# frgfm/Holocron

Hardware: NVIDIA H100
Metric: images/sec RepVGG-A0 224^2 bf16 train (higher is better)
Workload: dtype bf16

## Files before the change

### holocron_b200/_lib.py

```python
import ctypes
import os
from pathlib import Path
from typing import Optional

import torch

_LIB_PATH = Path(__file__).resolve().parent / "csrc" / "libholocron_b200.so"
_lib: Optional[ctypes.CDLL] = None

DTYPE_CODE = {torch.float32: 0, torch.bfloat16: 1, torch.float16: 2}


class HolocronB200Error(RuntimeError):
    pass


def lib_path() -> Path:
    return _LIB_PATH


SIGNATURES = {
    "hb_hard_mish_fwd": "ppzip",
    "hb_hard_mish_bwd": "pppzip",
    "hb_nl_relu_fwd": "ppzfip",
# ... 8 lines not shown
    "hb_conv2d_wgrad_acc_bf16": "ppppz" + "i" * 11 + "p",
    "hb_repvgg_wgrad_acc_bf16": "ppppppz" + "i" * 6 + "p",
    "hb_pack_conv_weights": "ppp" + "i" * 8 + "p",
    "hb_zero_insert_bf16": "pp" + "i" * 7 + "p",
    "hb_pack_conv_weights_multi": "ppip",
    "hb_pack_chunk_elems": "",
    "hb_pack_meta_bytes": "",
    "hb_conv2d_dgrad_s2_bf16": "ppppp" + "i" * 8 + "p",
    "hb_pack_dgrad_s2_weights": "pp" + "i" * 4 + "p",
    "hb_nchw_to_nhwc_pad_bf16": "pp" + "i" * 6 + "p",
    "hb_im2col_smallc_bf16": "pp" + "i" * 10 + "p",
    "hb_conv2d_fused_bf16": "ppp",
    "hb_conv_stat_slots_max": "",
    "hb_patch_stats_bf16": "pppp" + "i" * 10 + "fp",
    "hb_bn_stats_partials_bf16": "piippp",
    "hb_bn_stat_slots_max": "",
    "hb_bn_finalize": "ppppppp" + "pppp" + "iiiiffp",
    "hb_bn_partials_sums": "ppiiiipp",
    "hb_bn_finalize_sums": "p" * 10 + "iiiffp",
    "hb_bn_eval_affine": "ppppfiippppp",
    "hb_bn_act_fwd_bf16": "pppipppp" + "iiifi" + "ppp",
    "hb_bn_bwd_scratch_doubles": "iii",
    "hb_bn_act_bwd_bf16": "ppppi" + "pppppp" + "pppppp" + "pp" + "iiiifiip",
    "hb_bn_act_bwd_reduce_bf16": "ppppi" + "pppppp" + "pppp" + "iiiifip",
    "hb_bn_act_bwd_apply_bf16": "ppppi" + "pppppp" + "ppppp" + "iiifip",
    "hb_dwconv_fwd_bf16": "pppp" + "iiiiiiip",
    "hb_dwconv_bwd_data_bf16": "ppp" + "iiiiiiip",
    "hb_dwconv_wgrad_scratch_doubles": "ii",
    "hb_dwconv_bwd_weight_bf16": "ppppp" + "iiiiiiip",
    "hb_involution_fwd_bf16": "ppp" + "i" * 11 + "p",
# ... 138 lines not shown
```

### holocron_b200/csrc/bn_act.cu

```cuda
#include <cstdio>
#include <cstdlib>
#include <type_traits>
#include <utility>
#include "common.cuh"
#include "act.cuh"
#include "slab.cuh"

namespace {

using namespace hb;

constexpr int kThreads = kSlabThreads;
constexpr int kMaxBranches = 3;

struct Branches {
  const __nv_bfloat16* u[kMaxBranches];
  int n;
};

__device__ __forceinline__ void fold_stat_partials(const SlabGeo& g, const float* red, int C, float* parts) {
  fold_row_lanes<double, 2>(g, red, [&](int c, const double (&a)[2]) {
    *reinterpret_cast<float2*>(parts + ((size_t)blockIdx.x * C + c) * 2) = make_float2((float)a[0], (float)a[1]);
  });
}

__global__ void __launch_bounds__(kThreads) bn_stats_partials_kernel(const __nv_bfloat16* __restrict__ u, int M, int C,
                                                                     SlabGeo g, float* __restrict__ parts) {
  __shared__ float red[2][kThreads * 8];
  const auto [tx, ty, cg, active] = g.thread();
  float s[8], q[8];
#pragma unroll
  for (int j = 0; j < 8; ++j) { s[j] = 0.f; q[j] = 0.f; }
  if (active) {
    const size_t row_stride = (size_t)gridDim.x * g.rows_t;
    size_t m = (size_t)blockIdx.x * g.rows_t + ty;
    for (; m + row_stride < (size_t)M; m += 2 * row_stride) {
      float a[8], b[8];
      unpack8(ld16_stream(u + m * C + cg * 8), a);
      unpack8(ld16_stream(u + (m + row_stride) * C + cg * 8), b);
#pragma unroll
      for (int j = 0; j < 8; ++j) { s[j] += a[j] + b[j]; q[j] += a[j] * a[j] + b[j] * b[j]; }
    }
    if (m < (size_t)M) {
      float a[8];
      unpack8(ld16_stream(u + m * C + cg * 8), a);
#pragma unroll
      for (int j = 0; j < 8; ++j) { s[j] += a[j]; q[j] += a[j] * a[j]; }
    }
  }
#pragma unroll
  for (int j = 0; j < 8; ++j) { red[0][threadIdx.x * 8 + j] = s[j]; red[1][threadIdx.x * 8 + j] = q[j]; }
  __syncthreads();
  fold_stat_partials(g, &red[0][0], C, parts);
}

struct FinalizeParams {
  const float* parts[kMaxBranches];
  int slots[kMaxBranches];
  const float* gamma[kMaxBranches];
  const float* beta[kMaxBranches];
  float* running_mean[kMaxBranches];
  float* running_var[kMaxBranches];
  long long* num_batches_tracked[kMaxBranches];
  float* mean;
  float* rstd;
  float* scale;
  float* shift;
  int B, C, M;
// ... 137 lines not shown
  shift[c] = (beta ? beta[c] : 0.f) - rmean[c] * sc;
  if (mean) mean[c] = rmean[c];
  if (rstd) rstd[c] = r;
}

struct FwdParams {
  Branches br;
  const float* scale;
  const float* shift;
  const __nv_bfloat16* residual;
  __nv_bfloat16* out;
  int M, C, act;
  float slope;
  int res_after;
  float* out_stats;
};
using RawVec = Vec16<__nv_bfloat16>;

__device__ __forceinline__ void lds8(const float* p, float* f) {
  const float4 a = *reinterpret_cast<const float4*>(p);
  const float4 b = *reinterpret_cast<const float4*>(p + 4);
  f[0] = a.x; f[1] = a.y; f[2] = a.z; f[3] = a.w; f[4] = b.x; f[5] = b.y; f[6] = b.z; f[7] = b.w;
}

__host__ __device__ constexpr int ring_depth(int nt) { return nt <= 2 ? 7 : 3; }

__device__ __forceinline__ void cp_async16(uint32_t saddr, const void* g) {
  asm volatile("cp.async.cg.shared.global [%0], [%1], 16;" ::"r"(saddr), "l"(g) : "memory");
}
__device__ __forceinline__ void cp_async_commit() { asm volatile("cp.async.commit_group;" ::: "memory"); }
template <int N>
__device__ __forceinline__ void cp_async_wait() { asm volatile("cp.async.wait_group %0;" ::"n"(N) : "memory"); }
__device__ __forceinline__ RawVec lds16(uint32_t saddr) {
  RawVec r;
  asm volatile("ld.shared.v4.u32 {%0,%1,%2,%3}, [%4];" : "=r"(r.raw.x), "=r"(r.raw.y), "=r"(r.raw.z), "=r"(r.raw.w) : "r"(saddr));
  return r;
}
__device__ __forceinline__ uint32_t smem_addr(const void* p) { return (uint32_t)__cvta_generic_to_shared(p); }

template <int NT>
struct RowRing {
  static constexpr int kDepth = ring_depth(NT);
  static constexpr int kSlots = kDepth + 1;
  uint32_t base;
  size_t m0, stride, M;
  size_t col_off;
  int C;
  const __nv_bfloat16* src[NT > 0 ? NT : 1];
  __device__ __forceinline__ void init(uint8_t* smem, size_t m0_, size_t stride_, int M_, int C_, size_t col_off_) {
    base = smem_addr(smem) + threadIdx.x * 16;
    m0 = m0_; stride = stride_; M = (size_t)M_; col_off = col_off_; C = C_;
  }
  __device__ __forceinline__ uint32_t addr(int s, int t) const { return base + (uint32_t)((s * NT + t) * kThreads * 16); }
  __device__ __forceinline__ bool valid(size_t k) const { return m0 + k * stride < M; }
  __device__ __forceinline__ size_t off(size_t k) const { return (m0 + k * stride) * C + col_off; }
  __device__ __forceinline__ void issue(size_t k) const {
    if (valid(k)) {
      const int s = (int)(k % kSlots);
      const size_t o = off(k);
#pragma unroll
      for (int t = 0; t < NT; ++t)
        if (src[t]) cp_async16(addr(s, t), src[t] + o);
    }
    cp_async_commit();
  }
  __device__ __forceinline__ void prologue() const {
#pragma unroll
    for (int k = 0; k < kDepth; ++k) issue(k);
  }
  __device__ __forceinline__ void wait() const { cp_async_wait<kDepth - 1>(); }
};

template <int NB, bool kStats>
__global__ void __launch_bounds__(kThreads, 3) bn_act_fwd_kernel(FwdParams p, SlabGeo g) {
  extern __shared__ __align__(16) uint8_t ring_smem[];
  const auto [tx, ty, cg, active] = g.thread();
  float os[8], oq[8];
#pragma unroll
  for (int j = 0; j < 8; ++j) { os[j] = 0.f; oq[j] = 0.f; }
  __shared__ __align__(16) float k_sc[kMaxBranches][256];
  __shared__ __align__(16) float k_sh[256];
  {
    const int nch = g.cg_t * 8;
    for (int ch = threadIdx.x; ch < nch; ch += kThreads) {
      const int c = blockIdx.y * nch + ch;
      float shv = 0.f;
#pragma unroll
      for (int b = 0; b < NB; ++b) {
        k_sc[b][ch] = c < p.C ? p.scale[(size_t)b * p.C + c] : 0.f;
        shv += c < p.C ? p.shift[(size_t)b * p.C + c] : 0.f;
      }
      k_sh[ch] = shv;
    }
    __syncthreads();
  }
  if (!active && !kStats) return;
  if (active) {
    const bool has_res = p.residual != nullptr;
    RowRing<NB + 1> ring;
    ring.init(ring_smem, (size_t)blockIdx.x * g.rows_t + ty, (size_t)gridDim.x * g.rows_t, p.M, p.C, (size_t)cg * 8);
#pragma unroll
    for (int b = 0; b < NB; ++b) ring.src[b] = p.br.u[b];
    ring.src[NB] = p.residual;
    ring.prologue();
    for (size_t k = 0; ring.valid(k); ++k) {
      ring.wait();
      const int s = (int)(k % RowRing<NB + 1>::kSlots);
      RawVec u[NB > 0 ? NB : 1], r;
#pragma unroll
      for (int b = 0; b < NB; ++b) u[b] = lds16(ring.addr(s, b));
      if (has_res) r = lds16(ring.addr(s, NB));
      ring.issue(k + RowRing<NB + 1>::kDepth);
      float z[8];
      lds8(&k_sh[tx * 8], z);
#pragma unroll
      for (int b = 0; b < NB; ++b) {
        float f[8], sc[8];
        lds8(&k_sc[b][tx * 8], sc);
        unpack8(u[b], f);
#pragma unroll
        for (int j = 0; j < 8; ++j) z[j] = fmaf(sc[j], f[j], z[j]);
      }
      float rr[8];
      if (has_res) unpack8(r, rr);
      if (has_res && !p.res_after) {
        if (p.act == ACT_FRELU) {
#pragma unroll
          for (int j = 0; j < 8; ++j) z[j] = max_nan(z[j], rr[j]);
        } else {
#pragma unroll
          for (int j = 0; j < 8; ++j) z[j] += rr[j];
        }
      }
#pragma unroll
      for (int j = 0; j < 8; ++j) z[j] = act_fwd(p.act, z[j], p.slope);
      if (has_res && p.res_after) {
#pragma unroll
        for (int j = 0; j < 8; ++j) z[j] += rr[j];
      }
      Vec16<__nv_bfloat16> ov;
#pragma unroll
      for (int j = 0; j < 8; ++j) ov.v[j] = __float2bfloat16_rn(z[j]);
      st16(p.out + ring.off(k), ov);
      if (kStats) {
#pragma unroll
        for (int j = 0; j < 8; ++j) {
          const float f = __bfloat162float(ov.v[j]);
          os[j] += f; oq[j] = fmaf(f, f, oq[j]);
        }
      }
    }
  }
  if (!kStats) return;
  cp_async_wait<0>();
  __syncthreads();
  float* red = reinterpret_cast<float*>(ring_smem);
#pragma unroll
  for (int j = 0; j < 8; ++j) {
    red[threadIdx.x * 8 + j] = active ? os[j] : 0.f;
    red[kThreads * 8 + threadIdx.x * 8 + j] = active ? oq[j] : 0.f;
  }
  __syncthreads();
  fold_stat_partials(g, red, p.C, p.out_stats);
}

struct BwdParams {
  Branches br;
  const __nv_bfloat16* dout;
  const __nv_bfloat16* residual;
  const float* scale;
  const float* shift;
  const float* mean;
  const float* rstd;
  double* sums;
  double* part;
  const double* count;
  __nv_bfloat16* du[kMaxBranches];
  __nv_bfloat16* dres;
  int M, C, act;
  float slope;
  int train;
  int res_after;
};

struct SlabConsts {
  float scale[kMaxBranches][256];
  float cu[kMaxBranches][256];
  float c0[kMaxBranches][256];
  float shift[256];
};
// ... 56 lines not shown
#pragma unroll
      for (int j = 0; j < 8; ++j) {
        const float gate = z[j] > r[j] ? 1.f : (z[j] == r[j] ? 0.5f : 0.f);
        dz[j] = d[j] * gate;
        dr[j] = d[j] - dz[j];
      }
      return;
    }
#pragma unroll
    for (int j = 0; j < 8; ++j) z[j] += r[j];
  }
#pragma unroll
  for (int j = 0; j < 8; ++j) { dz[j] = d[j] * act_grad(p.act, z[j], p.slope); dr[j] = dz[j]; }
}

template <int NB>
__device__ __forceinline__ void init_bwd_ring(RowRing<NB + 2>& ring, const BwdParams& p, const SlabGeo& g, uint8_t* ring_smem,
                                              int ty, int cg) {
  ring.init(ring_smem, (size_t)blockIdx.x * g.rows_t + ty, (size_t)gridDim.x * g.rows_t, p.M, p.C, (size_t)cg * 8);
#pragma unroll
  for (int b = 0; b < NB; ++b) ring.src[b] = p.br.u[b];
  ring.src[NB] = (p.residual && !p.res_after) ? p.residual : nullptr;
  ring.src[NB + 1] = p.dout;
}

template <int NB>
__global__ void __launch_bounds__(kThreads, 2) bn_act_bwd_reduce_kernel(BwdParams p, SlabGeo g) {
  extern __shared__ __align__(16) uint8_t dyn_smem[];
  SlabConsts& k = *reinterpret_cast<SlabConsts*>(dyn_smem);
  float* red = reinterpret_cast<float*>(dyn_smem + sizeof(SlabConsts));
  uint8_t* ring_smem = dyn_smem + sizeof(SlabConsts) + kThreads * 8 * sizeof(float);
  load_slab_consts<NB>(k, p, g, false);
  const auto [tx, ty, cg, active] = g.thread();
  float acc[1 + NB][8];
#pragma unroll
  for (int i = 0; i < 1 + NB; ++i)
#pragma unroll
    for (int j = 0; j < 8; ++j) acc[i][j] = 0.f;
  if (active) {
    RowRing<NB + 2> ring;
    init_bwd_ring<NB>(ring, p, g, ring_smem, ty, cg);
    ring.prologue();
    for (size_t kk = 0; ring.valid(kk); ++kk) {
      ring.wait();
      const int s = (int)(kk % RowRing<NB + 2>::kSlots);
      RawVec uv[NB > 0 ? NB : 1], rv, dv;
#pragma unroll
      for (int b = 0; b < NB; ++b) uv[b] = lds16(ring.addr(s, b));
      if (ring.src[NB]) rv = lds16(ring.addr(s, NB));
      dv = lds16(ring.addr(s, NB + 1));
      ring.issue(kk + RowRing<NB + 2>::kDepth);
      float u[NB > 0 ? NB : 1][8], dz[8], dr[8];
      recompute_dz<NB>(p, k, tx * 8, uv, rv, dv, u, dz, dr);
#pragma unroll
      for (int j = 0; j < 8; ++j) acc[0][j] += dz[j];
#pragma unroll
      for (int b = 0; b < NB; ++b) {
#pragma unroll
        for (int j = 0; j < 8; ++j) acc[1 + b][j] = fmaf(dz[j], u[b][j], acc[1 + b][j]);
      }
    }
  }
#pragma unroll
  for (int i = 0; i < 1 + NB; ++i) {
    __syncthreads();
#pragma unroll
    for (int j = 0; j < 8; ++j) red[threadIdx.x * 8 + j] = acc[i][j];
    __syncthreads();
    fold_row_lanes<double, 1>(g, red, [&](int c, const double (&a)[1]) {
      p.part[((size_t)blockIdx.x * (1 + NB) + i) * p.C + c] = a[0];
    });
  }
}

template <int NB>
__global__ void __launch_bounds__(kThreads, 2) bn_act_bwd_apply_kernel(BwdParams p, SlabGeo g) {
  extern __shared__ __align__(16) uint8_t dyn_smem[];
  SlabConsts& k = *reinterpret_cast<SlabConsts*>(dyn_smem);
  uint8_t* ring_smem = dyn_smem + sizeof(SlabConsts);
  load_slab_consts<NB>(k, p, g, true);
  const auto [tx, ty, cg, active] = g.thread();
  if (!active) return;
  RowRing<NB + 2> ring;
  init_bwd_ring<NB>(ring, p, g, ring_smem, ty, cg);
  ring.prologue();
  for (size_t kk = 0; ring.valid(kk); ++kk) {
    ring.wait();
    const int s = (int)(kk % RowRing<NB + 2>::kSlots);
    RawVec uv[NB > 0 ? NB : 1], rv, dv;
#pragma unroll
    for (int b = 0; b < NB; ++b) uv[b] = lds16(ring.addr(s, b));
    if (ring.src[NB]) rv = lds16(ring.addr(s, NB));
    dv = lds16(ring.addr(s, NB + 1));
    ring.issue(kk + RowRing<NB + 2>::kDepth);
    const size_t off = ring.off(kk);
    float u[NB > 0 ? NB : 1][8], dz[8], dr[8];
    recompute_dz<NB>(p, k, tx * 8, uv, rv, dv, u, dz, dr);
    if (p.dres) store8(p.dres + off, dr);
#pragma unroll
    for (int b = 0; b < NB; ++b) {
      if (p.du[b]) {
        float sc[8], cu[8], c0[8], d[8];
        lds8(&k.scale[b][tx * 8], sc);
        lds8(&k.cu[b][tx * 8], cu);
        lds8(&k.c0[b][tx * 8], c0);
#pragma unroll
        for (int j = 0; j < 8; ++j) d[j] = fmaf(sc[j], dz[j], fmaf(cu[j], u[b][j], c0[j]));
        store8(p.du[b] + off, d);
      }
// ... 24 lines not shown
    const float db = (float)tot[0];
    if (p.dgamma) p.dgamma[o] = dg;
    if (p.dbeta) p.dbeta[o] = db;
    if (c < p.C_logical) {
      if (p.gacc[b]) p.gacc[b][c] += dg;
      if (p.bacc[b]) p.bacc[b][c] += db;
    }
  }
}

inline int env_int(const char* name, int dflt) {
  const char* v = getenv(name);
  return v ? atoi(v) : dflt;
}

template <typename K>
inline int resident_blocks(K kernel, size_t smem) {
  int n = 0;
  if (cudaOccupancyMaxActiveBlocksPerMultiprocessor(&n, kernel, kThreads, smem) != cudaSuccess || n < 1) n = 1;
  return n;
}

template <auto Kernel>
std::pair<decltype(Kernel), int> instance(size_t smem) {
  static int occ = 0;
  if (!occ) {
    if (cudaFuncSetAttribute(Kernel, cudaFuncAttributeMaxDynamicSharedMemorySize, 200 * 1024) != cudaSuccess) return {Kernel, 0};
    occ = resident_blocks(Kernel, smem);
  }
  return {Kernel, occ};
}

template <typename F>
auto with_nb(int B, F pick) {
  switch (B) {
    case 0: return pick(std::integral_constant<int, 0>{});
    case 1: return pick(std::integral_constant<int, 1>{});
    case 2: return pick(std::integral_constant<int, 2>{});
    default: return pick(std::integral_constant<int, 3>{});
  }
}

inline size_t ring_bytes(int tensors) { return (size_t)(ring_depth(tensors) + 1) * tensors * kThreads * 16; }

inline int finalize_params(FinalizeParams& p, const float* const* parts, const int* slots, const float* const* gamma,
                           const float* const* beta, float* const* running_mean, float* const* running_var,
                           long long* const* num_batches_tracked, int B) {
  if (B < 1 || B > kMaxBranches) return (int)cudaErrorInvalidValue;
  for (int b = 0; b < B; ++b) {
    if (parts) {
      if (!parts[b] || !slots || slots[b] < 1) return (int)cudaErrorInvalidValue;
      p.parts[b] = parts[b];
      p.slots[b] = slots[b];
    }
    p.gamma[b] = gamma ? gamma[b] : nullptr;
    p.beta[b] = beta ? beta[b] : nullptr;
    p.running_mean[b] = running_mean ? running_mean[b] : nullptr;
    p.running_var[b] = running_var ? running_var[b] : nullptr;
// ... 12 lines not shown
  p.dout = (const __nv_bfloat16*)dout; p.residual = (const __nv_bfloat16*)residual;
  p.scale = scale; p.shift = shift; p.mean = mean; p.rstd = rstd;
  p.sums = scratch; p.part = scratch + (size_t)(1 + B) * C; p.count = count;
  p.du[0] = (__nv_bfloat16*)du0; p.du[1] = (__nv_bfloat16*)du1; p.du[2] = (__nv_bfloat16*)du2;
  p.dres = (__nv_bfloat16*)dres;
  p.M = M; p.C = C; p.act = act; p.slope = slope; p.train = train; p.res_after = res_after;
  return p;
}

inline int launch_bwd_reduce(const BwdParams& p, float* dgamma, float* dbeta, float* const* gamma_grad_acc,
                             float* const* beta_grad_acc, int C_logical, cudaStream_t st) {
  const int B = p.br.n, C = p.C;
  const SlabGeo g = SlabGeo::make(C);
  static const int cap_red_env = env_int("HB_BN_CAP_RED", 0);
  static const bool use_occ = env_int("HB_BN_USE_OCC", 1) != 0, occ_debug = env_int("HB_BN_DEBUG", 0) != 0;
  int cap_red = cap_red_env > 0 ? cap_red_env : (B <= 1 ? 3 : 2);
  if (cap_red > 3) cap_red = 3;
  const size_t smem = sizeof(SlabConsts) + kThreads * 8 * sizeof(float) + ring_bytes(B + 2);
  const auto [kernel, occ] = with_nb(B, [&](auto nb) { return instance<bn_act_bwd_reduce_kernel<decltype(nb)::value>>(smem); });
  if (!occ) return (int)cudaErrorInvalidValue;
  if (occ_debug) fprintf(stderr, "[hb] bn_act_bwd_reduce_kernel<%d> smem %zu: %d resident blocks/SM (cap %d)\n", B, smem, occ, cap_red);
  const dim3 grid = g.grid(p.M, (use_occ && occ < cap_red) ? occ : cap_red);
  kernel<<<grid, kThreads, smem, st>>>(p, g);
  HB_LAUNCH_CHECK();
  BwdFinalizeParams f{};
  f.part = p.part; f.sums = p.sums; f.mean = p.mean; f.rstd = p.rstd; f.dgamma = dgamma; f.dbeta = dbeta;
  for (int b = 0; b < B; ++b) {
    f.gacc[b] = gamma_grad_acc ? gamma_grad_acc[b] : nullptr;
    f.bacc[b] = beta_grad_acc ? beta_grad_acc[b] : nullptr;
  }
  f.nblocks = (int)grid.x; f.B = B; f.C = C; f.C_logical = C_logical > 0 ? C_logical : C;
  bn_bwd_finalize_kernel<<<(C + kFinCh - 1) / kFinCh, dim3(kFinCh, kFinLanes), 0, st>>>(f);
  HB_LAUNCH_CHECK();
  return 0;
}

inline int launch_bwd_apply(const BwdParams& p, cudaStream_t st) {
  const int B = p.br.n;
  const SlabGeo g = SlabGeo::make(p.C);
  static const int cap_app_env = env_int("HB_BN_CAP_APPLY", 0);
  static const bool use_occ = env_int("HB_BN_USE_OCC", 1) != 0, occ_debug = env_int("HB_BN_DEBUG", 0) != 0;
  const int cap_app = cap_app_env > 0 ? cap_app_env : (B <= 2 ? 3 : 2);
  const size_t smem = sizeof(SlabConsts) + ring_bytes(B + 2);
  const auto [kernel, occ] = with_nb(B, [&](auto nb) { return instance<bn_act_bwd_apply_kernel<decltype(nb)::value>>(smem); });
  if (!occ) return (int)cudaErrorInvalidValue;
  if (occ_debug) fprintf(stderr, "[hb] bn_act_bwd_apply_kernel<%d> smem %zu: %d resident blocks/SM (cap %d)\n", B, smem, occ, cap_app);
  const dim3 grid = g.grid(p.M, (use_occ && occ < cap_app) ? occ : cap_app);
  kernel<<<grid, kThreads, smem, st>>>(p, g);
  HB_LAUNCH_CHECK();
  return 0;
}

}

extern "C" {

int hb_bn_stats_partials_bf16(const void* u, int M, int C, float* parts, int* slots, void* stream) {
  if (C % 8 != 0 || !slots) return (int)cudaErrorInvalidValue;
  const SlabGeo g = SlabGeo::make(C);
  static const int min_rows = env_int("HB_BN_STATS_ROWS", 16);
  const dim3 grid = g.grid(M, 4, min_rows);
  *slots = (int)grid.x;
  bn_stats_partials_kernel<<<grid, kThreads, 0, (cudaStream_t)stream>>>((const __nv_bfloat16*)u, M, C, g, parts);
  HB_LAUNCH_CHECK();
  return 0;
}

int hb_bn_stat_slots_max(void) { return HB_NUM_SMS * 8; }

int hb_bn_finalize(const float* const* parts, const int* slots, const float* const* gamma, const float* const* beta,
                   float* const* running_mean, float* const* running_var, long long* const* num_batches_tracked,
                   float* mean, float* rstd, float* scale, float* shift, int B, int C, int C_logical, int M, float eps,
                   float momentum, void* stream) {
  FinalizeParams p{};
  if (!parts) return (int)cudaErrorInvalidValue;
  if (const int rc = finalize_params(p, parts, slots, gamma, beta, running_mean, running_var, num_batches_tracked, B))
    return rc;
  p.mean = mean; p.rstd = rstd; p.scale = scale; p.shift = shift;
  p.C = C; p.M = M; p.C_logical = C_logical; p.eps = eps; p.momentum = momentum;
  bn_finalize_kernel<<<dim3((C + kFinCh - 1) / kFinCh, B), dim3(kFinCh, kFinLanes), 0, (cudaStream_t)stream>>>(p);
  HB_LAUNCH_CHECK();
  return 0;
}
// ... 36 lines not shown

int hb_bn_act_fwd_bf16(const void* u0, const void* u1, const void* u2, int B, const float* scale, const float* shift,
                       const void* residual, void* out, int M, int C, int act, float slope, int res_after,
                       float* out_stats, int* out_stat_slots, void* stream) {
  if (C % 8 != 0 || B < 0 || B > kMaxBranches) return (int)cudaErrorInvalidValue;
  FwdParams p{};
  p.br = Branches{{(const __nv_bfloat16*)u0, (const __nv_bfloat16*)u1, (const __nv_bfloat16*)u2}, B};
  p.scale = scale; p.shift = shift; p.residual = (const __nv_bfloat16*)residual; p.out = (__nv_bfloat16*)out;
  p.M = M; p.C = C; p.act = act; p.slope = slope; p.res_after = res_after;
  if (out_stats && !out_stat_slots) return (int)cudaErrorInvalidValue;
  p.out_stats = out_stats;
  const SlabGeo g = SlabGeo::make(C);
  static const int per_sm_env = env_int("HB_BN_CAP_FWD", 0);
  static const bool use_occ = env_int("HB_BN_USE_OCC", 1) != 0, occ_debug = env_int("HB_BN_DEBUG", 0) != 0;
  cudaStream_t st = (cudaStream_t)stream;
  const size_t smem = ring_bytes(B + 1);
  const auto [kernel, occ] = with_nb(B, [&](auto nb) {
    constexpr int NB = decltype(nb)::value;
    return out_stats ? instance<bn_act_fwd_kernel<NB, true>>(smem) : instance<bn_act_fwd_kernel<NB, false>>(smem);
  });
  if (!occ) return (int)cudaErrorInvalidValue;
  if (occ_debug)
    fprintf(stderr, "[hb] bn_act_fwd_kernel<%d,%d> smem %zu: %d resident blocks/SM\n", B, (int)(out_stats != nullptr), smem, occ);
  const int fixed = (B + (residual != nullptr) >= 3) ? 3 : 4;
  const int per_sm = per_sm_env > 0 ? (per_sm_env < 4 ? per_sm_env : 4) : (use_occ ? (occ < 4 ? occ : 4) : fixed);
  const dim3 grid = g.grid(M, per_sm);
  if (out_stat_slots) *out_stat_slots = (int)grid.x;
  kernel<<<grid, kThreads, smem, st>>>(p, g);
  HB_LAUNCH_CHECK();
  return 0;
}

size_t hb_bn_bwd_scratch_doubles(int M, int C, int B) {
  const SlabGeo g = SlabGeo::make(C);
  const dim3 grid = g.grid(M, 3);
  return (size_t)(1 + B) * C * (1 + (size_t)grid.x);
}

int hb_bn_act_bwd_bf16(const void* dout, const void* u0, const void* u1, const void* u2, int B, const float* scale,
                       const float* shift, const float* mean, const float* rstd, const void* residual, double* scratch,
                       void* du0, void* du1, void* du2, void* dres, float* dgamma, float* dbeta,
                       float* const* gamma_grad_acc, float* const* beta_grad_acc, int C_logical, int M, int C, int act,
// ... 35 lines not shown
```

### holocron_b200/nn/_fused.py

```python
import ctypes
import functools
import os
import weakref
from typing import List, Optional, Sequence, Tuple

import torch
import torch.distributed as dist
from torch import Tensor, nn

from .._lib import DTYPE_CODE, ConvArgs, check, dtype_code, lib, ptr, require_cuda, stream_ptr

ACT_NONE, ACT_RELU, ACT_RELU6, ACT_SILU, ACT_LEAKY, ACT_MISH, ACT_HARDMISH, ACT_FRELU = range(8)

_c_float = ctypes.c_float
_VP3 = ctypes.c_void_p * 3

KERNEL_TIMER = None


def _timed(kind: str, info: dict, fn):
    if KERNEL_TIMER is None:
        return fn()
    e0, e1 = torch.cuda.Event(enable_timing=True), torch.cuda.Event(enable_timing=True)
    e0.record()
# ... 499 lines not shown


_I3 = ctypes.c_int * 3


def _elem_bytes_info(kind: str, m: int, c: int, reads: int, writes: int) -> dict:
    return dict(shape=(kind, m, c, reads, writes), launches=1, flops=0.0, bytes=2.0 * m * c * (reads + writes))


def _bn_batch_stats(us: Sequence[Tensor], branches, g32, b32, stats: Tensor, c: int, c_log: int, m: int,
                    group=None) -> Optional[Tensor]:
    if m == 1 and group is None:
        raise ValueError(f"Expected more than 1 value per channel when training, got input size {us[0].shape}")
    L = lib()
    nb = len(us)
    parts, slots = [], []
    for u in us:
        st = get_stats(u)
        if st is None:
            buf = torch.empty((bn_stat_slots(u.device), c, 2), device=u.device, dtype=torch.float32)
            sl = ctypes.c_int(0)
            check(_timed("bn_stats", _elem_bytes_info("bn_stats", m, c, 1, 0), lambda: L.hb_bn_stats_partials_bf16(
                ptr(u), m, c, ptr(buf), ctypes.byref(sl), stream_ptr())), "hb_bn_stats_partials_bf16")
            st = (buf, sl.value)
        parts.append(st[0])
        slots.append(st[1])
    eps, mom = branches[0].eps, branches[0].momentum
    if any(b.eps != eps or b.momentum != mom for b in branches):
        raise NotImplementedError("branches with different eps/momentum")
    track = [b.track_running_stats for b in branches]
    if mom is None and any(track):
        raise NotImplementedError("cumulative moving average (momentum=None)")
    running = (_arr3([b.running_mean if t else None for b, t in zip(branches, track)]),
               _arr3([b.running_var if t else None for b, t in zip(branches, track)]),
               _arr3([b.num_batches_tracked if t else None for b, t in zip(branches, track)]))
    outs = (ptr(stats[0]), ptr(stats[1]), ptr(stats[2]), ptr(stats[3]))
    if group is None:
        check(L.hb_bn_finalize(_arr3(parts), _I3(*(slots + [0] * (3 - nb))), _arr3(g32), _arr3(b32), *running, *outs, nb, c,
                               c_log, m, _c_float(eps), _c_float(0.0 if mom is None else mom), stream_ptr()),
              "hb_bn_finalize")
        return None
# ... 412 lines not shown
```

### include/holocron_b200.h

```cpp
#ifndef HOLOCRON_B200_H
#define HOLOCRON_B200_H

#include <stddef.h>

#ifdef __cplusplus
extern "C" {
#endif

int hb_hard_mish_fwd(const void* x, void* y, size_t n, int dtype, void* stream);
int hb_hard_mish_bwd(const void* x, const void* dy, void* dx, size_t n, int dtype, void* stream);
int hb_nl_relu_fwd(const void* x, void* y, size_t n, float beta, int dtype, void* stream);
int hb_nl_relu_bwd(const void* x, const void* dy, void* dx, size_t n, float beta, int dtype, void* stream);
int hb_nl_relu_bwd_from_out(const void* y, const void* dy, void* dx, size_t n, float beta, int dtype, void* stream);

int hb_conv2d_fprop_bf16(const void* x, const void* w, void* y, const float* bias, const void* residual, int N, int H,
                         int W, int Cin, int Cout, int R, int S, int stride, int pad, int dil, int act, int num_ctas,
                         void* stream);
typedef struct hb_conv_args {
  const void* x; const void* w; void* y; const float* bias; const void* residual;
  int N, H, W, Cin, Cout, R, S, stride, pad, dil, act, num_ctas;
  const void* xe; const void* we; int Ce;
  const void* w2; void* y2;
  float* stats; float* stats2;
  const float* norm_mean; const float* norm_rstd; const float* norm_wsum;
// ... 19 lines not shown
int hb_pack_conv_weights(const float* w, void* wf, void* wd, int Cout, int Cin, int R, int S, int CinP, int CinD,
                         int CoutP, int CoutF, void* stream);
int hb_pack_conv_weights_multi(const void* metas, const void* chunks, int num_chunks, void* stream);
int hb_pack_chunk_elems(void);
int hb_pack_meta_bytes(void);
int hb_conv2d_dgrad_s2_bf16(const void* dy, const void* wcls, const void* dy1, const void* wd1, void* dx, int N, int H, int W,
                            int Ho, int Wo, int C, int Cd, int num_ctas, void* stream);
int hb_pack_dgrad_s2_weights(const float* w, void* out, int Cout, int Cin, int CinD, int CoutP, void* stream);
int hb_zero_insert_bf16(const void* x, void* y, int N, int Hi, int Wi, int Ho, int Wo, int C, int sp, void* stream);
int hb_nchw_to_nhwc_pad_bf16(const void* x, void* y, int N, int C, int H, int W, int CP, int dtype, void* stream);

int hb_im2col_smallc_bf16(const void* x, void* col, int N, int C, int H, int W, int R, int S, int stride, int pad, int Kp,
                          int dtype, void* stream);

int hb_bn_stats_partials_bf16(const void* u, int M, int C, float* parts, int* slots, void* stream);
int hb_bn_stat_slots_max(void);
int hb_bn_finalize(const float* const* parts, const int* slots, const float* const* gamma, const float* const* beta,
                   float* const* running_mean, float* const* running_var, long long* const* num_batches_tracked,
                   float* mean, float* rstd, float* scale, float* shift, int B, int C, int C_logical, int M, float eps,
                   float momentum, void* stream);
int hb_bn_partials_sums(const float* const* parts, const int* slots, int B, int C, int C_logical, int M, double* sums,
                        void* stream);
int hb_bn_finalize_sums(const double* sums, const float* const* gamma, const float* const* beta,
                        float* const* running_mean, float* const* running_var, long long* const* num_batches_tracked,
                        float* mean, float* rstd, float* scale, float* shift, int B, int C, int C_logical, float eps,
                        float momentum, void* stream);
int hb_bn_eval_affine(const float* gamma, const float* beta, const float* running_mean, const float* running_var,
                      float eps, int C, int C_logical, float* scale, float* shift, float* mean, float* rstd,
                      void* stream);
int hb_bn_act_fwd_bf16(const void* u0, const void* u1, const void* u2, int B, const float* scale, const float* shift,
                       const void* residual, void* out, int M, int C, int act, float slope, int res_after,
// ... 211 lines not shown
```

Baseline: 9305.

## Batch BN stats across branches and decouple logical row blocks from grid size

Replaces the per-branch BN stats launches with one multi-tensor kernel that grid-strides over (branch, row-block) items. The fwd-stats and bwd-reduce kernels now walk a fixed count of logical row blocks, so the partial-sum layout no longer depends on how many blocks the grid holds. Ring-buffer depths and launch bounds are now tuned per branch count, and the apply kernel issues its ring prologue before loading slab constants. It also adds a forced-row-block override for testing. The aims are fewer launches, better occupancy, and more prefetch overlap, at the cost of extra loop and sync overhead inside blocks.

Measured after the change: 9309 (median of 6 runs). Within noise of the previous version (+0.1%).

```diff
diff --git a/holocron_b200/_lib.py b/holocron_b200/_lib.py
--- a/holocron_b200/_lib.py
+++ b/holocron_b200/_lib.py
@@ -46,6 +46,8 @@
     "hb_conv_stat_slots_max": "",
     "hb_patch_stats_bf16": "pppp" + "i" * 10 + "fp",
     "hb_bn_stats_partials_bf16": "piippp",
+    "hb_bn_stats_partials_multi_bf16": "piiippp",
+    "hb_bn_force_row_blocks": "i",
     "hb_bn_stat_slots_max": "",
     "hb_bn_finalize": "ppppppp" + "pppp" + "iiiiffp",
     "hb_bn_partials_sums": "ppiiiipp",
diff --git a/holocron_b200/csrc/bn_act.cu b/holocron_b200/csrc/bn_act.cu
--- a/holocron_b200/csrc/bn_act.cu
+++ b/holocron_b200/csrc/bn_act.cu
@@ -18,40 +18,62 @@
   int n;
 };
 
-__device__ __forceinline__ void fold_stat_partials(const SlabGeo& g, const float* red, int C, float* parts) {
+__device__ __forceinline__ void fold_stat_partials(const SlabGeo& g, const float* red, int C, int slot, float* parts) {
   fold_row_lanes<double, 2>(g, red, [&](int c, const double (&a)[2]) {
-    *reinterpret_cast<float2*>(parts + ((size_t)blockIdx.x * C + c) * 2) = make_float2((float)a[0], (float)a[1]);
+    *reinterpret_cast<float2*>(parts + ((size_t)slot * C + c) * 2) = make_float2((float)a[0], (float)a[1]);
   });
 }
 
-__global__ void __launch_bounds__(kThreads) bn_stats_partials_kernel(const __nv_bfloat16* __restrict__ u, int M, int C,
-                                                                     SlabGeo g, float* __restrict__ parts) {
-  __shared__ float red[2][kThreads * 8];
+constexpr int kStatsPerSm = 4, kStatsMinRows = 16;
+constexpr int kFwdStatsPerSm[kMaxBranches + 1] = {4, 3, 3, 3};
+constexpr int kReducePerSm[kMaxBranches + 1] = {2, 3, 2, 2};
+
+struct StatsParams {
+  const __nv_bfloat16* u[kMaxBranches];
+  float* parts[kMaxBranches];
+  int n, M, C, L;
+};
+__device__ __forceinline__ void stats_block(const StatsParams& p, const SlabGeo& g, int t, int lb, float* red);
+
+__global__ void __launch_bounds__(kThreads) bn_stats_partials_kernel(StatsParams p, SlabGeo g) {
+  __shared__ float red[2 * kThreads * 8];
+  for (int i = blockIdx.x; i < p.n * p.L; i += gridDim.x) {
+    stats_block(p, g, i / p.L, i % p.L, red);
+    __syncthreads();
+  }
+}
+
+__device__ __forceinline__ void stats_block(const StatsParams& p, const SlabGeo& g, int t, int lb, float* red) {
+  const __nv_bfloat16* __restrict__ u = t == 0 ? p.u[0] : (t == 1 ? p.u[1] : p.u[2]);
+  float* parts = t == 0 ? p.parts[0] : (t == 1 ? p.parts[1] : p.parts[2]);
+  const int C = p.C;
+  const size_t M = (size_t)p.M;
   const auto [tx, ty, cg, active] = g.thread();
   float s[8], q[8];
 #pragma unroll
   for (int j = 0; j < 8; ++j) { s[j] = 0.f; q[j] = 0.f; }
   if (active) {
-    const size_t row_stride = (size_t)gridDim.x * g.rows_t;
-    size_t m = (size_t)blockIdx.x * g.rows_t + ty;
-    for (; m + row_stride < (size_t)M; m += 2 * row_stride) {
+    const size_t row_stride = (size_t)p.L * g.rows_t;
+    const __nv_bfloat16* col = u + cg * 8;
+    size_t m = (size_t)lb * g.rows_t + ty;
+    for (; m + row_stride < M; m += 2 * row_stride) {
       float a[8], b[8];
-      unpack8(ld16_stream(u + m * C + cg * 8), a);
-      unpack8(ld16_stream(u + (m + row_stride) * C + cg * 8), b);
+      unpack8(ld16_stream(col + m * C), a);
+      unpack8(ld16_stream(col + (m + row_stride) * C), b);
 #pragma unroll
       for (int j = 0; j < 8; ++j) { s[j] += a[j] + b[j]; q[j] += a[j] * a[j] + b[j] * b[j]; }
     }
-    if (m < (size_t)M) {
+    if (m < M) {
       float a[8];
-      unpack8(ld16_stream(u + m * C + cg * 8), a);
+      unpack8(ld16_stream(col + m * C), a);
 #pragma unroll
       for (int j = 0; j < 8; ++j) { s[j] += a[j]; q[j] += a[j] * a[j]; }
     }
   }
 #pragma unroll
-  for (int j = 0; j < 8; ++j) { red[0][threadIdx.x * 8 + j] = s[j]; red[1][threadIdx.x * 8 + j] = q[j]; }
+  for (int j = 0; j < 8; ++j) { red[threadIdx.x * 8 + j] = s[j]; red[kThreads * 8 + threadIdx.x * 8 + j] = q[j]; }
   __syncthreads();
-  fold_stat_partials(g, &red[0][0], C, parts);
+  fold_stat_partials(g, red, C, lb, parts);
 }
 
 struct FinalizeParams {
@@ -219,6 +241,7 @@
   float slope;
   int res_after;
   float* out_stats;
+  int L;
 };
 using RawVec = Vec16<__nv_bfloat16>;
 
@@ -228,7 +251,9 @@
   f[0] = a.x; f[1] = a.y; f[2] = a.z; f[3] = a.w; f[4] = b.x; f[5] = b.y; f[6] = b.z; f[7] = b.w;
 }
 
-__host__ __device__ constexpr int ring_depth(int nt) { return nt <= 2 ? 7 : 3; }
+constexpr int kFwdDepth[kMaxBranches + 1] = {7, 7, 4, 3};
+constexpr int kReduceDepth[kMaxBranches + 1] = {7, 3, 4, 3};
+constexpr int kApplyDepth[kMaxBranches + 1] = {7, 4, 5, 4};
 
 __device__ __forceinline__ void cp_async16(uint32_t saddr, const void* g) {
   asm volatile("cp.async.cg.shared.global [%0], [%1], 16;" ::"r"(saddr), "l"(g) : "memory");
@@ -243,9 +268,9 @@
 }
 __device__ __forceinline__ uint32_t smem_addr(const void* p) { return (uint32_t)__cvta_generic_to_shared(p); }
 
-template <int NT>
+template <int NT, int Depth>
 struct RowRing {
-  static constexpr int kDepth = ring_depth(NT);
+  static constexpr int kDepth = Depth;
   static constexpr int kSlots = kDepth + 1;
   uint32_t base;
   size_t m0, stride, M;
@@ -258,10 +283,11 @@
   }
   __device__ __forceinline__ uint32_t addr(int s, int t) const { return base + (uint32_t)((s * NT + t) * kThreads * 16); }
   __device__ __forceinline__ bool valid(size_t k) const { return m0 + k * stride < M; }
+  __device__ __forceinline__ static int slot(size_t k) { return (int)((uint32_t)k % (uint32_t)kSlots); }
   __device__ __forceinline__ size_t off(size_t k) const { return (m0 + k * stride) * C + col_off; }
   __device__ __forceinline__ void issue(size_t k) const {
     if (valid(k)) {
-      const int s = (int)(k % kSlots);
+      const int s = slot(k);
       const size_t o = off(k);
 #pragma unroll
       for (int t = 0; t < NT; ++t)
@@ -277,7 +303,7 @@
 };
 
 template <int NB, bool kStats>
-__global__ void __launch_bounds__(kThreads, 3) bn_act_fwd_kernel(FwdParams p, SlabGeo g) {
+__global__ void __launch_bounds__(kThreads, NB == 0 && kStats ? 4 : 3) bn_act_fwd_kernel(FwdParams p, SlabGeo g) {
   extern __shared__ __align__(16) uint8_t ring_smem[];
   const auto [tx, ty, cg, active] = g.thread();
   float os[8], oq[8];
@@ -300,73 +326,78 @@
     __syncthreads();
   }
   if (!active && !kStats) return;
-  if (active) {
-    const bool has_res = p.residual != nullptr;
-    RowRing<NB + 1> ring;
-    ring.init(ring_smem, (size_t)blockIdx.x * g.rows_t + ty, (size_t)gridDim.x * g.rows_t, p.M, p.C, (size_t)cg * 8);
-#pragma unroll
-    for (int b = 0; b < NB; ++b) ring.src[b] = p.br.u[b];
-    ring.src[NB] = p.residual;
-    ring.prologue();
-    for (size_t k = 0; ring.valid(k); ++k) {
-      ring.wait();
-      const int s = (int)(k % RowRing<NB + 1>::kSlots);
-      RawVec u[NB > 0 ? NB : 1], r;
-#pragma unroll
-      for (int b = 0; b < NB; ++b) u[b] = lds16(ring.addr(s, b));
-      if (has_res) r = lds16(ring.addr(s, NB));
-      ring.issue(k + RowRing<NB + 1>::kDepth);
-      float z[8];
-      lds8(&k_sh[tx * 8], z);
-#pragma unroll
-      for (int b = 0; b < NB; ++b) {
-        float f[8], sc[8];
-        lds8(&k_sc[b][tx * 8], sc);
-        unpack8(u[b], f);
-#pragma unroll
-        for (int j = 0; j < 8; ++j) z[j] = fmaf(sc[j], f[j], z[j]);
-      }
-      float rr[8];
-      if (has_res) unpack8(r, rr);
-      if (has_res && !p.res_after) {
-        if (p.act == ACT_FRELU) {
-#pragma unroll
-          for (int j = 0; j < 8; ++j) z[j] = max_nan(z[j], rr[j]);
-        } else {
+  for (int lb = blockIdx.x; lb < p.L; lb += gridDim.x) {
+    if (active) {
+      const bool has_res = p.residual != nullptr;
+      using Ring = RowRing<NB + 1, kFwdDepth[NB]>;
+      Ring ring;
+      ring.init(ring_smem, (size_t)lb * g.rows_t + ty, (size_t)p.L * g.rows_t, p.M, p.C, (size_t)cg * 8);
+#pragma unroll
+      for (int b = 0; b < NB; ++b) ring.src[b] = p.br.u[b];
+      ring.src[NB] = p.residual;
+      ring.prologue();
+      for (size_t k = 0; ring.valid(k); ++k) {
+        ring.wait();
+        const int s = Ring::slot(k);
+        RawVec u[NB > 0 ? NB : 1], r;
+#pragma unroll
+        for (int b = 0; b < NB; ++b) u[b] = lds16(ring.addr(s, b));
+        if (has_res) r = lds16(ring.addr(s, NB));
+        ring.issue(k + Ring::kDepth);
+        float z[8];
+        lds8(&k_sh[tx * 8], z);
+#pragma unroll
+        for (int b = 0; b < NB; ++b) {
+          float f[8], sc[8];
+          lds8(&k_sc[b][tx * 8], sc);
+          unpack8(u[b], f);
+#pragma unroll
+          for (int j = 0; j < 8; ++j) z[j] = fmaf(sc[j], f[j], z[j]);
+        }
+        float rr[8];
+        if (has_res) unpack8(r, rr);
+        if (has_res && !p.res_after) {
+          if (p.act == ACT_FRELU) {
+#pragma unroll
+            for (int j = 0; j < 8; ++j) z[j] = max_nan(z[j], rr[j]);
+          } else {
+#pragma unroll
+            for (int j = 0; j < 8; ++j) z[j] += rr[j];
+          }
+        }
+#pragma unroll
+        for (int j = 0; j < 8; ++j) z[j] = act_fwd(p.act, z[j], p.slope);
+        if (has_res && p.res_after) {
 #pragma unroll
           for (int j = 0; j < 8; ++j) z[j] += rr[j];
         }
-      }
-#pragma unroll
-      for (int j = 0; j < 8; ++j) z[j] = act_fwd(p.act, z[j], p.slope);
-      if (has_res && p.res_after) {
-#pragma unroll
-        for (int j = 0; j < 8; ++j) z[j] += rr[j];
-      }
-      Vec16<__nv_bfloat16> ov;
-#pragma unroll
-      for (int j = 0; j < 8; ++j) ov.v[j] = __float2bfloat16_rn(z[j]);
-      st16(p.out + ring.off(k), ov);
-      if (kStats) {
-#pragma unroll
-        for (int j = 0; j < 8; ++j) {
-          const float f = __bfloat162float(ov.v[j]);
-          os[j] += f; oq[j] = fmaf(f, f, oq[j]);
+        Vec16<__nv_bfloat16> ov;
+#pragma unroll
+        for (int j = 0; j < 8; ++j) ov.v[j] = __float2bfloat16_rn(z[j]);
+        st16(p.out + ring.off(k), ov);
+        if (kStats) {
+#pragma unroll
+          for (int j = 0; j < 8; ++j) {
+            const float f = __bfloat162float(ov.v[j]);
+            os[j] += f; oq[j] = fmaf(f, f, oq[j]);
+          }
         }
       }
     }
-  }
-  if (!kStats) return;
-  cp_async_wait<0>();
-  __syncthreads();
-  float* red = reinterpret_cast<float*>(ring_smem);
-#pragma unroll
-  for (int j = 0; j < 8; ++j) {
-    red[threadIdx.x * 8 + j] = active ? os[j] : 0.f;
-    red[kThreads * 8 + threadIdx.x * 8 + j] = active ? oq[j] : 0.f;
-  }
-  __syncthreads();
-  fold_stat_partials(g, red, p.C, p.out_stats);
+    if (!kStats) continue;
+    cp_async_wait<0>();
+    __syncthreads();
+    float* red = reinterpret_cast<float*>(ring_smem);
+#pragma unroll
+    for (int j = 0; j < 8; ++j) {
+      red[threadIdx.x * 8 + j] = active ? os[j] : 0.f;
+      red[kThreads * 8 + threadIdx.x * 8 + j] = active ? oq[j] : 0.f;
+      os[j] = 0.f; oq[j] = 0.f;
+    }
+    __syncthreads();
+    fold_stat_partials(g, red, p.C, lb, p.out_stats);
+    __syncthreads();
+  }
 }
 
 struct BwdParams {
@@ -379,6 +410,7 @@
   const float* rstd;
   double* sums;
   double* part;
+  int L;
   const double* count;
   __nv_bfloat16* du[kMaxBranches];
   __nv_bfloat16* dres;
@@ -465,10 +497,10 @@
   for (int j = 0; j < 8; ++j) { dz[j] = d[j] * act_grad(p.act, z[j], p.slope); dr[j] = dz[j]; }
 }
 
-template <int NB>
-__device__ __forceinline__ void init_bwd_ring(RowRing<NB + 2>& ring, const BwdParams& p, const SlabGeo& g, uint8_t* ring_smem,
-                                              int ty, int cg) {
-  ring.init(ring_smem, (size_t)blockIdx.x * g.rows_t + ty, (size_t)gridDim.x * g.rows_t, p.M, p.C, (size_t)cg * 8);
+template <int NB, typename Ring>
+__device__ __forceinline__ void init_bwd_ring(Ring& ring, const BwdParams& p, const SlabGeo& g, uint8_t* ring_smem,
+                                              int ty, int cg, int lb, int nblocks) {
+  ring.init(ring_smem, (size_t)lb * g.rows_t + ty, (size_t)nblocks * g.rows_t, p.M, p.C, (size_t)cg * 8);
 #pragma unroll
   for (int b = 0; b < NB; ++b) ring.src[b] = p.br.u[b];
   ring.src[NB] = (p.residual && !p.res_after) ? p.residual : nullptr;
@@ -476,51 +508,55 @@
 }
 
 template <int NB>
-__global__ void __launch_bounds__(kThreads, 2) bn_act_bwd_reduce_kernel(BwdParams p, SlabGeo g) {
+__global__ void __launch_bounds__(kThreads, NB == 1 ? 3 : 2) bn_act_bwd_reduce_kernel(BwdParams p, SlabGeo g) {
   extern __shared__ __align__(16) uint8_t dyn_smem[];
   SlabConsts& k = *reinterpret_cast<SlabConsts*>(dyn_smem);
   float* red = reinterpret_cast<float*>(dyn_smem + sizeof(SlabConsts));
   uint8_t* ring_smem = dyn_smem + sizeof(SlabConsts) + kThreads * 8 * sizeof(float);
   load_slab_consts<NB>(k, p, g, false);
   const auto [tx, ty, cg, active] = g.thread();
-  float acc[1 + NB][8];
-#pragma unroll
-  for (int i = 0; i < 1 + NB; ++i)
-#pragma unroll
-    for (int j = 0; j < 8; ++j) acc[i][j] = 0.f;
-  if (active) {
-    RowRing<NB + 2> ring;
-    init_bwd_ring<NB>(ring, p, g, ring_smem, ty, cg);
-    ring.prologue();
-    for (size_t kk = 0; ring.valid(kk); ++kk) {
-      ring.wait();
-      const int s = (int)(kk % RowRing<NB + 2>::kSlots);
-      RawVec uv[NB > 0 ? NB : 1], rv, dv;
-#pragma unroll
-      for (int b = 0; b < NB; ++b) uv[b] = lds16(ring.addr(s, b));
-      if (ring.src[NB]) rv = lds16(ring.addr(s, NB));
-      dv = lds16(ring.addr(s, NB + 1));
-      ring.issue(kk + RowRing<NB + 2>::kDepth);
-      float u[NB > 0 ? NB : 1][8], dz[8], dr[8];
-      recompute_dz<NB>(p, k, tx * 8, uv, rv, dv, u, dz, dr);
-#pragma unroll
-      for (int j = 0; j < 8; ++j) acc[0][j] += dz[j];
-#pragma unroll
-      for (int b = 0; b < NB; ++b) {
-#pragma unroll
-        for (int j = 0; j < 8; ++j) acc[1 + b][j] = fmaf(dz[j], u[b][j], acc[1 + b][j]);
+  for (int lb = blockIdx.x; lb < p.L; lb += gridDim.x) {
+    float acc[1 + NB][8];
+#pragma unroll
+    for (int i = 0; i < 1 + NB; ++i)
+#pragma unroll
+      for (int j = 0; j < 8; ++j) acc[i][j] = 0.f;
+    if (active) {
+      using Ring = RowRing<NB + 2, kReduceDepth[NB]>;
+      Ring ring;
+      init_bwd_ring<NB>(ring, p, g, ring_smem, ty, cg, lb, p.L);
+      ring.prologue();
+      for (size_t kk = 0; ring.valid(kk); ++kk) {
+        ring.wait();
+        const int s = Ring::slot(kk);
+        RawVec uv[NB > 0 ? NB : 1], rv, dv;
+#pragma unroll
+        for (int b = 0; b < NB; ++b) uv[b] = lds16(ring.addr(s, b));
+        if (ring.src[NB]) rv = lds16(ring.addr(s, NB));
+        dv = lds16(ring.addr(s, NB + 1));
+        ring.issue(kk + Ring::kDepth);
+        float u[NB > 0 ? NB : 1][8], dz[8], dr[8];
+        recompute_dz<NB>(p, k, tx * 8, uv, rv, dv, u, dz, dr);
+#pragma unroll
+        for (int j = 0; j < 8; ++j) acc[0][j] += dz[j];
+#pragma unroll
+        for (int b = 0; b < NB; ++b) {
+#pragma unroll
+          for (int j = 0; j < 8; ++j) acc[1 + b][j] = fmaf(dz[j], u[b][j], acc[1 + b][j]);
+        }
       }
     }
-  }
-#pragma unroll
-  for (int i = 0; i < 1 + NB; ++i) {
+#pragma unroll
+    for (int i = 0; i < 1 + NB; ++i) {
+      __syncthreads();
+#pragma unroll
+      for (int j = 0; j < 8; ++j) red[threadIdx.x * 8 + j] = acc[i][j];
+      __syncthreads();
+      fold_row_lanes<double, 1>(g, red, [&](int c, const double (&a)[1]) {
+        p.part[((size_t)lb * (1 + NB) + i) * p.C + c] = a[0];
+      });
+    }
     __syncthreads();
-#pragma unroll
-    for (int j = 0; j < 8; ++j) red[threadIdx.x * 8 + j] = acc[i][j];
-    __syncthreads();
-    fold_row_lanes<double, 1>(g, red, [&](int c, const double (&a)[1]) {
-      p.part[((size_t)blockIdx.x * (1 + NB) + i) * p.C + c] = a[0];
-    });
   }
 }
 
@@ -529,21 +565,24 @@
   extern __shared__ __align__(16) uint8_t dyn_smem[];
   SlabConsts& k = *reinterpret_cast<SlabConsts*>(dyn_smem);
   uint8_t* ring_smem = dyn_smem + sizeof(SlabConsts);
+  const auto [tx, ty, cg, active] = g.thread();
+  using Ring = RowRing<NB + 2, kApplyDepth[NB]>;
+  Ring ring;
+  if (active) {
+    init_bwd_ring<NB>(ring, p, g, ring_smem, ty, cg, blockIdx.x, gridDim.x);
+    ring.prologue();
+  }
   load_slab_consts<NB>(k, p, g, true);
-  const auto [tx, ty, cg, active] = g.thread();
   if (!active) return;
-  RowRing<NB + 2> ring;
-  init_bwd_ring<NB>(ring, p, g, ring_smem, ty, cg);
-  ring.prologue();
   for (size_t kk = 0; ring.valid(kk); ++kk) {
     ring.wait();
-    const int s = (int)(kk % RowRing<NB + 2>::kSlots);
+    const int s = Ring::slot(kk);
     RawVec uv[NB > 0 ? NB : 1], rv, dv;
 #pragma unroll
     for (int b = 0; b < NB; ++b) uv[b] = lds16(ring.addr(s, b));
     if (ring.src[NB]) rv = lds16(ring.addr(s, NB));
     dv = lds16(ring.addr(s, NB + 1));
-    ring.issue(kk + RowRing<NB + 2>::kDepth);
+    ring.issue(kk + Ring::kDepth);
     const size_t off = ring.off(kk);
     float u[NB > 0 ? NB : 1][8], dz[8], dr[8];
     recompute_dz<NB>(p, k, tx * 8, uv, rv, dv, u, dz, dr);
@@ -598,6 +637,23 @@
   return v ? atoi(v) : dflt;
 }
 
+int g_forced_row_blocks = 0;
+
+inline int logical_row_blocks(const SlabGeo& g, int M, int per_sm, int min_rows = 4) {
+  return (int)g.grid(M, per_sm, min_rows).x;
+}
+
+inline dim3 walk_grid(const SlabGeo& g, int L, int per_sm) {
+  const int n = g_forced_row_blocks > 0 ? g_forced_row_blocks : g.max_blocks(per_sm);
+  return dim3((unsigned)(n < L ? n : L), (unsigned)g.slabs);
+}
+
+inline dim3 free_grid(const SlabGeo& g, int M, int per_sm) {
+  dim3 grid = g.grid(M, per_sm);
+  if (g_forced_row_blocks > 0) grid.x = (unsigned)g_forced_row_blocks;
+  return grid;
+}
+
 template <typename K>
 inline int resident_blocks(K kernel, size_t smem) {
   int n = 0;
@@ -625,7 +681,7 @@
   }
 }
 
-inline size_t ring_bytes(int tensors) { return (size_t)(ring_depth(tensors) + 1) * tensors * kThreads * 16; }
+inline size_t ring_bytes(int tensors, int depth) { return (size_t)(depth + 1) * tensors * kThreads * 16; }
 
 inline int finalize_params(FinalizeParams& p, const float* const* parts, const int* slots, const float* const* gamma,
                            const float* const* beta, float* const* running_mean, float* const* running_var,
@@ -668,14 +724,15 @@
   const SlabGeo g = SlabGeo::make(C);
   static const int cap_red_env = env_int("HB_BN_CAP_RED", 0);
   static const bool use_occ = env_int("HB_BN_USE_OCC", 1) != 0, occ_debug = env_int("HB_BN_DEBUG", 0) != 0;
-  int cap_red = cap_red_env > 0 ? cap_red_env : (B <= 1 ? 3 : 2);
-  if (cap_red > 3) cap_red = 3;
-  const size_t smem = sizeof(SlabConsts) + kThreads * 8 * sizeof(float) + ring_bytes(B + 2);
+  const int cap_red = cap_red_env > 0 ? cap_red_env : (B <= 1 ? 3 : 2);
+  const size_t smem = sizeof(SlabConsts) + kThreads * 8 * sizeof(float) + ring_bytes(B + 2, kReduceDepth[B]);
   const auto [kernel, occ] = with_nb(B, [&](auto nb) { return instance<bn_act_bwd_reduce_kernel<decltype(nb)::value>>(smem); });
   if (!occ) return (int)cudaErrorInvalidValue;
   if (occ_debug) fprintf(stderr, "[hb] bn_act_bwd_reduce_kernel<%d> smem %zu: %d resident blocks/SM (cap %d)\n", B, smem, occ, cap_red);
-  const dim3 grid = g.grid(p.M, (use_occ && occ < cap_red) ? occ : cap_red);
-  kernel<<<grid, kThreads, smem, st>>>(p, g);
+  BwdParams pr = p;
+  pr.L = logical_row_blocks(g, p.M, kReducePerSm[B]);
+  const dim3 grid = walk_grid(g, pr.L, (use_occ && occ < cap_red) ? occ : cap_red);
+  kernel<<<grid, kThreads, smem, st>>>(pr, g);
   HB_LAUNCH_CHECK();
   BwdFinalizeParams f{};
   f.part = p.part; f.sums = p.sums; f.mean = p.mean; f.rstd = p.rstd; f.dgamma = dgamma; f.dbeta = dbeta;
@@ -683,7 +740,7 @@
     f.gacc[b] = gamma_grad_acc ? gamma_grad_acc[b] : nullptr;
     f.bacc[b] = beta_grad_acc ? beta_grad_acc[b] : nullptr;
   }
-  f.nblocks = (int)grid.x; f.B = B; f.C = C; f.C_logical = C_logical > 0 ? C_logical : C;
+  f.nblocks = pr.L; f.B = B; f.C = C; f.C_logical = C_logical > 0 ? C_logical : C;
   bn_bwd_finalize_kernel<<<(C + kFinCh - 1) / kFinCh, dim3(kFinCh, kFinLanes), 0, st>>>(f);
   HB_LAUNCH_CHECK();
   return 0;
@@ -695,11 +752,11 @@
   static const int cap_app_env = env_int("HB_BN_CAP_APPLY", 0);
   static const bool use_occ = env_int("HB_BN_USE_OCC", 1) != 0, occ_debug = env_int("HB_BN_DEBUG", 0) != 0;
   const int cap_app = cap_app_env > 0 ? cap_app_env : (B <= 2 ? 3 : 2);
-  const size_t smem = sizeof(SlabConsts) + ring_bytes(B + 2);
+  const size_t smem = sizeof(SlabConsts) + ring_bytes(B + 2, kApplyDepth[B]);
   const auto [kernel, occ] = with_nb(B, [&](auto nb) { return instance<bn_act_bwd_apply_kernel<decltype(nb)::value>>(smem); });
   if (!occ) return (int)cudaErrorInvalidValue;
   if (occ_debug) fprintf(stderr, "[hb] bn_act_bwd_apply_kernel<%d> smem %zu: %d resident blocks/SM (cap %d)\n", B, smem, occ, cap_app);
-  const dim3 grid = g.grid(p.M, (use_occ && occ < cap_app) ? occ : cap_app);
+  const dim3 grid = free_grid(g, p.M, (use_occ && occ < cap_app) ? occ : cap_app);
   kernel<<<grid, kThreads, smem, st>>>(p, g);
   HB_LAUNCH_CHECK();
   return 0;
@@ -709,18 +766,38 @@
 
 extern "C" {
 
-int hb_bn_stats_partials_bf16(const void* u, int M, int C, float* parts, int* slots, void* stream) {
-  if (C % 8 != 0 || !slots) return (int)cudaErrorInvalidValue;
+int hb_bn_stats_partials_multi_bf16(const void* const* us, int n, int M, int C, float* const* parts, int* slots,
+                                    void* stream) {
+  if (C % 8 != 0 || !slots || !us || !parts || n < 1 || n > kMaxBranches) return (int)cudaErrorInvalidValue;
+  StatsParams p{};
+  for (int t = 0; t < n; ++t) {
+    if (!us[t] || !parts[t]) return (int)cudaErrorInvalidValue;
+    p.u[t] = (const __nv_bfloat16*)us[t];
+    p.parts[t] = parts[t];
+  }
   const SlabGeo g = SlabGeo::make(C);
-  static const int min_rows = env_int("HB_BN_STATS_ROWS", 16);
-  const dim3 grid = g.grid(M, 4, min_rows);
-  *slots = (int)grid.x;
-  bn_stats_partials_kernel<<<grid, kThreads, 0, (cudaStream_t)stream>>>((const __nv_bfloat16*)u, M, C, g, parts);
+  p.n = n; p.M = M; p.C = C;
+  p.L = logical_row_blocks(g, M, kStatsPerSm, kStatsMinRows);
+  const int items = n * p.L;
+  const dim3 grid((unsigned)(g_forced_row_blocks > 0 && g_forced_row_blocks < items ? g_forced_row_blocks : items),
+                  (unsigned)g.slabs);
+  *slots = p.L;
+  bn_stats_partials_kernel<<<grid, kThreads, 0, (cudaStream_t)stream>>>(p, g);
   HB_LAUNCH_CHECK();
   return 0;
 }
 
+int hb_bn_stats_partials_bf16(const void* u, int M, int C, float* parts, int* slots, void* stream) {
+  return hb_bn_stats_partials_multi_bf16(&u, 1, M, C, &parts, slots, stream);
+}
+
 int hb_bn_stat_slots_max(void) { return HB_NUM_SMS * 8; }
+
+int hb_bn_force_row_blocks(int n) {
+  if (n < 0) return (int)cudaErrorInvalidValue;
+  g_forced_row_blocks = n;
+  return 0;
+}
 
 int hb_bn_finalize(const float* const* parts, const int* slots, const float* const* gamma, const float* const* beta,
                    float* const* running_mean, float* const* running_var, long long* const* num_batches_tracked,
@@ -787,7 +864,7 @@
   static const int per_sm_env = env_int("HB_BN_CAP_FWD", 0);
   static const bool use_occ = env_int("HB_BN_USE_OCC", 1) != 0, occ_debug = env_int("HB_BN_DEBUG", 0) != 0;
   cudaStream_t st = (cudaStream_t)stream;
-  const size_t smem = ring_bytes(B + 1);
+  const size_t smem = ring_bytes(B + 1, kFwdDepth[B]);
   const auto [kernel, occ] = with_nb(B, [&](auto nb) {
     constexpr int NB = decltype(nb)::value;
     return out_stats ? instance<bn_act_fwd_kernel<NB, true>>(smem) : instance<bn_act_fwd_kernel<NB, false>>(smem);
@@ -796,9 +873,16 @@
   if (occ_debug)
     fprintf(stderr, "[hb] bn_act_fwd_kernel<%d,%d> smem %zu: %d resident blocks/SM\n", B, (int)(out_stats != nullptr), smem, occ);
   const int fixed = (B + (residual != nullptr) >= 3) ? 3 : 4;
-  const int per_sm = per_sm_env > 0 ? (per_sm_env < 4 ? per_sm_env : 4) : (use_occ ? (occ < 4 ? occ : 4) : fixed);
-  const dim3 grid = g.grid(M, per_sm);
-  if (out_stat_slots) *out_stat_slots = (int)grid.x;
+  const int per_sm = per_sm_env > 0 ? per_sm_env : (use_occ ? (occ < 4 ? occ : 4) : fixed);
+  dim3 grid;
+  if (out_stats) {
+    p.L = logical_row_blocks(g, M, kFwdStatsPerSm[B]);
+    grid = walk_grid(g, p.L, per_sm);
+  } else {
+    grid = free_grid(g, M, per_sm);
+    p.L = (int)grid.x;
+  }
+  if (out_stat_slots) *out_stat_slots = p.L;
   kernel<<<grid, kThreads, smem, st>>>(p, g);
   HB_LAUNCH_CHECK();
   return 0;
diff --git a/holocron_b200/nn/_fused.py b/holocron_b200/nn/_fused.py
--- a/holocron_b200/nn/_fused.py
+++ b/holocron_b200/nn/_fused.py
@@ -537,17 +537,19 @@
         raise ValueError(f"Expected more than 1 value per channel when training, got input size {us[0].shape}")
     L = lib()
     nb = len(us)
-    parts, slots = [], []
-    for u in us:
-        st = get_stats(u)
-        if st is None:
-            buf = torch.empty((bn_stat_slots(u.device), c, 2), device=u.device, dtype=torch.float32)
-            sl = ctypes.c_int(0)
-            check(_timed("bn_stats", _elem_bytes_info("bn_stats", m, c, 1, 0), lambda: L.hb_bn_stats_partials_bf16(
-                ptr(u), m, c, ptr(buf), ctypes.byref(sl), stream_ptr())), "hb_bn_stats_partials_bf16")
-            st = (buf, sl.value)
-        parts.append(st[0])
-        slots.append(st[1])
+    sts = [get_stats(u) for u in us]
+    missing = [i for i, st in enumerate(sts) if st is None]
+    if missing:
+        bufs = [torch.empty((bn_stat_slots(us[i].device), c, 2), device=us[i].device, dtype=torch.float32) for i in missing]
+        sl = ctypes.c_int(0)
+        check(_timed("bn_stats", _elem_bytes_info("bn_stats", m, c, len(missing), 0),
+                     lambda: L.hb_bn_stats_partials_multi_bf16(_arr3([us[i] for i in missing]), len(missing), m, c,
+                                                               _arr3(bufs), ctypes.byref(sl), stream_ptr())),
+              "hb_bn_stats_partials_multi_bf16")
+        for i, buf in zip(missing, bufs):
+            sts[i] = (buf, sl.value)
+    parts = [st[0] for st in sts]
+    slots = [st[1] for st in sts]
     eps, mom = branches[0].eps, branches[0].momentum
     if any(b.eps != eps or b.momentum != mom for b in branches):
         raise NotImplementedError("branches with different eps/momentum")
diff --git a/include/holocron_b200.h b/include/holocron_b200.h
--- a/include/holocron_b200.h
+++ b/include/holocron_b200.h
@@ -57,7 +57,10 @@
                           int dtype, void* stream);
 
 int hb_bn_stats_partials_bf16(const void* u, int M, int C, float* parts, int* slots, void* stream);
+int hb_bn_stats_partials_multi_bf16(const void* const* us, int n, int M, int C, float* const* parts, int* slots,
+                                    void* stream);
 int hb_bn_stat_slots_max(void);
+int hb_bn_force_row_blocks(int n);
 int hb_bn_finalize(const float* const* parts, const int* slots, const float* const* gamma, const float* const* beta,
                    float* const* running_mean, float* const* running_var, long long* const* num_batches_tracked,
                    float* mean, float* rstd, float* scale, float* shift, int B, int C, int C_logical, int M, float eps,
```
